# j-moralejo-pinas/dist_classicrl

Hardware: AMD Instinct MI355X
Metric: env-steps/sec at 128 agents, 1e6x16 Q-table; 1/2/4/8 GPU + HBM GB/s %peak (higher is better)
Workload: dtype f32

## Files before the change

dist_classicrl_amd/csrc/qe_rollout_df.h:

```cpp
#pragma once
#include "qe_rollout_lane.h"

namespace qe {

constexpr int DF_CAP = 128;
constexpr int DF_WT = 4096;
constexpr uint32_t DF_EMPTY = 0xFFFFFFFFu;
constexpr int64_t DF_MAX_STATES = 1ll << 25;
constexpr int DF_SPIN_LIMIT = 1 << 18;
constexpr unsigned ERR_DF_TIMEOUT = 5u;

struct M128 {
    unsigned long long lo, hi;
};
__device__ __forceinline__ M128 m128_zero() { return M128{0ull, 0ull}; }
__device__ __forceinline__ bool m128_any(const M128& a) { return (a.lo | a.hi) != 0ull; }
__device__ __forceinline__ M128 m128_and(const M128& a, const M128& b) { return M128{a.lo & b.lo, a.hi & b.hi}; }
__device__ __forceinline__ M128 m128_andnot(const M128& a, const M128& b) { return M128{a.lo & ~b.lo, a.hi & ~b.hi}; }
__device__ __forceinline__ M128 m128_or(const M128& a, const M128& b) { return M128{a.lo | b.lo, a.hi | b.hi}; }
__device__ __forceinline__ M128 m128_bit(int i) {
    return M128{i < 64 ? 1ull << i : 0ull, i >= 64 ? 1ull << (i - 64) : 0ull};
}
__device__ __forceinline__ M128 m128_below(int i) {
    return M128{i < 64 ? (1ull << i) - 1ull : ~0ull, i > 64 ? (1ull << (i - 64)) - 1ull : 0ull};
// ... 152 lines not shown
    const int tid = threadIdx.x;
    const int n_main = (int)((c.N + 63) & ~63ll);
    const int wave_tid = __builtin_amdgcn_readfirstlane(tid);
    const bool helper = wave_tid >= n_main;
    const int n_waves = n_main >> 6;
    const int i = helper ? tid - n_main : (tid & 63) * n_waves + (tid >> 6);
    const bool active = FULL ? !helper : (!helper && i < c.N);
    const int ii = i < c.N ? i : 0;
    Pending<T> p;
    p.n = helper ? 0 : c.n[ii];
    p.aux = c.aux[ii];
    p.s = 0; p.a = 0; p.pred = 0; p.r = 0.0f; p.term = false;
    float acc = c.acc[ii];
    unsigned long long dep_total = 0, ep_base = 0;
    unsigned extra_rounds = 0;
    int w_next = WT, w_cur = WT, w_prev = WT;
    int own_next = DF_CAP, own_cur = DF_CAP, own_prev = DF_CAP;
    const int flush_every = 32;
    int flush_in = flush_every;
    for (int k = tid; k < 4 * (WT + 1); k += (int)blockDim.x) (&lds.key[0][0])[k] = DF_EMPTY;
    for (int k = tid; k < 4 * (DF_CAP + 1) * 4; k += (int)blockDim.x) (&lds.wmask[0][0][0])[k] = 0u;
    for (int k = tid; k < 2 * DF_CAP; k += (int)blockDim.x) df_pub_write(&lds.pub[0][0] + k, 0u, (T)0, 0);
    static_assert(sizeof(Ctx<T>) <= sizeof(lds.cold), "context stash too small");
    if (tid == 0) {
        *reinterpret_cast<Ctx<T>*>(lds.cold) = c;
        lds.ep_n = 0u; lds.abort_ = 0u; lds.stat_dep = 0u; lds.stat_rounds = 0u;
        c.ctrl->error = 0u;
        c.ctrl->inv_count = 0u;
    }
    __syncthreads();
    const M128 my_bit = m128_bit(ii), below = m128_below(ii);
    const bool nan_sel = c.nan_select != 0;

    auto advance = [&](const RowV<T, NV>& row, M valid, long long t1, const U4& x, unsigned long long thr_t1, bool row_nan) {
        const bool explore = (unsigned long long)x.x < thr_t1;
        T picked;
        int act = select_lane<T, NV, M>(masked_row<MASKED>(row, valid), valid, explore, x.y, x.z, &picked, nan_sel && row_nan);
        if (act < 0) {
            c.ctrl->error = ERR_EMPTY_CHOICE;
            act = 0;
        }
        const int32_t n = p.n;
        const Transition tr = Env::step(ev, i, n, p.aux, act, c.step0 + (unsigned long long)t1);
        p.s = n; p.a = act; p.pred = picked; p.r = tr.reward; p.term = tr.terminated; p.n = tr.next_obs;
        lds.pub_a[t1 & 3][ii] = (unsigned char)act;
    };
    auto philox_of = [&](long long t1) {
        const unsigned long long step1 = c.step0 + (unsigned long long)t1;
        return philox4x32_10(c.agent_offset + (uint32_t)ii, (uint32_t)step1, (uint32_t)(step1 >> 32), STREAM_POLICY,
                             c.seed_lo, c.seed_hi);
    };
    auto draws = [&](long long t1) {
        const int slot = (int)(t1 & 1);
        return U4{lds.draws[slot][0][ii], lds.draws[slot][1][ii], lds.draws[slot][2][ii], 0u};
    };
    auto produce = [&](long long t1) {
        const U4 x = philox_of(t1);
        const int slot = (int)(t1 & 1);
        lds.draws[slot][0][ii] = x.x; lds.draws[slot][1][ii] = x.y; lds.draws[slot][2][ii] = x.z;
    };

    M128 Ws = my_bit;
    M128 Wn = m128_zero();
    M128 Wst = m128_zero();
    auto bookkeeping = [&](long long k, bool first) {
        uint32_t* const key_w = lds.key[(k + 1) & 3];
        const uint32_t* const key_r = lds.key[k & 3];
        const uint32_t* const key_st = lds.key[(k + 3) & 3];
        const uint32_t rowid = (uint32_t)p.n;
        const uint32_t mine = (rowid << 7) | (uint32_t)ii;
// ... 8 lines not shown
             odd_st = k_st != DF_EMPTY && (k_st >> 7) != rowid;
        while (__any(odd_w || odd_r || odd_st)) {
            h_w = odd_w ? (h_w + 1) & (WT - 1) : h_w;
            h_r = (h_r + 1) & (WT - 1);
            h_st = (h_st + 1) & (WT - 1);
            const uint32_t o2 = atomicCAS(&key_w[odd_w ? h_w : WT], odd_w ? DF_EMPTY : DF_EMPTY - 1u, mine);
            const uint32_t r2 = key_r[odd_r ? h_r : WT];
            const uint32_t s2 = key_st[odd_st ? h_st : WT];
            o_w = odd_w ? o2 : o_w; k_r = odd_r ? r2 : k_r; k_st = odd_st ? s2 : k_st;
            odd_w = o_w != DF_EMPTY && (o_w >> 7) != rowid; odd_r = k_r != DF_EMPTY && (k_r >> 7) != rowid;
            odd_st = k_st != DF_EMPTY && (k_st >> 7) != rowid;
        }
        const int own_w = o_w == DF_EMPTY ? ii : (int)(o_w & 127u);
        atomicOr(&lds.wmask[(k + 1) & 3][own_w][ii >> 5], 1u << (ii & 31));
        const bool found_r = k_r != DF_EMPTY, found_st = k_st != DF_EMPTY;
        Wn = m128_zero();
        Wst = m128_zero();
        if (__any(found_r || found_st)) {
            const M128 mr = lds_mask_load(lds.wmask[k & 3][found_r ? (int)(k_r & 127u) : DF_CAP]);
            const M128 ms = lds_mask_load(lds.wmask[(k + 3) & 3][found_st ? (int)(k_st & 127u) : DF_CAP]);
            if (found_r) Wn = mr;
            if (found_st) Wst = ms;
        }
        w_prev = w_cur; w_cur = w_next; w_next = h_w;
        own_prev = own_cur; own_cur = own_next; own_next = own_w;
    };

    RowV<T, NV> row;
    RowV<T, NV> row_next;
    {
        load_row_lane<NV>(row, c.q, p.n);
        if (active) {
            const M valid0 = valid_mask_lane<Env, NV, MASKED>(ev, i, p.n);
            advance(row, valid0, 0, philox_of(0), c.thr[0], row_nan_lane<NV>(masked_row<MASKED>(row, valid0)));
            const uint32_t rowid = (uint32_t)p.s, mine = (rowid << 7) | (uint32_t)ii;
            int h = (int)(mix32(rowid) & (WT - 1));
            uint32_t old = atomicCAS(&lds.key[0][h], DF_EMPTY, mine);
            while (old != DF_EMPTY && (old >> 7) != rowid) {
                h = (h + 1) & (WT - 1);
                old = atomicCAS(&lds.key[0][h], DF_EMPTY, mine);
            }
            own_next = old == DF_EMPTY ? ii : (int)(old & 127u);
            atomicOr(&lds.wmask[0][own_next][ii >> 5], 1u << (ii & 31));
            w_next = h;
        }
        if (helper) produce(1);
        __syncthreads();
        if (active) bookkeeping(0, true);
        load_row_lane<NV>(row_next, c.q, p.n);
        asm volatile("" ::: "memory");
        c.pred[ii] = (T)0;
        if constexpr (LEAN == 2) reinterpret_cast<DeltaEntry*>(c.pred)[ii] = DeltaEntry{0u, 0.0f};
    }
    __syncthreads();
    DeltaEntry* dl = c.dlog ? c.dlog + c.dlog_base + ii : nullptr;
    const long long dl_steps = c.dlog ? (c.dlog_cap - c.dlog_base) / c.N : 0;
    double lr_t = c.lr[0];
    unsigned long long thr_t1 = c.thr[steps > 1 ? 1 : 0];
    int vzero;
    asm volatile("v_mov_b32 %0, 0" : "=v"(vzero));
    bool timed_out = false;
    for (long long t = 0; t < steps; ++t) {
        const bool last = t + 1 == steps;
        const bool dl_ok = t < dl_steps;
        QL_STAMP(7);
        const U4 x = draws(t + 1);
        if (helper && !last) produce(t + 2);
        const uint32_t stamp = ((uint32_t)t + 1u) & 0xFFFFFFu, stamp_prev = (uint32_t)t & 0xFFFFFFu;
        const int par = (int)(t & 1);
        const M valid = valid_mask_lane<Env, NV, MASKED>(ev, ii, p.n);
        if constexpr (LEAN == 2) asm volatile("s_waitcnt vmcnt(2)" ::: "memory");
        else asm volatile("s_waitcnt vmcnt(1)" ::: "memory");
        df_take_row<T, NV>(row, row_next);
        const double lr_next = ((const double*)(uintptr_t)c.lr)[(last ? t : t + 1) + vzero];
        const unsigned long long thr_next = ((const unsigned long long*)(uintptr_t)c.thr)[(t + 2 < steps ? t + 2 : steps - 1) + vzero];
        const bool company = active && (m128_any(m128_andnot(Ws, my_bit)) || m128_any(Wn) || m128_any(Wst));
        const bool any_company = __any(company);
        const bool self_loop = p.n == p.s;
        const float r_t = p.r;
        const bool term_t = p.term;
        const int64_t cell = (int64_t)p.s * (4 * NV) + p.a;
        T q1 = 0, u = 0;
        bool row_nan = false;
        bool dep_u = false;
        bool is_last = active;
        QL_STAMP(0);
        float u_t = 0.0f;
        unsigned ep_raw = 0;
        unsigned long long enders = 0;
        float ep_value = 0.0f;
        auto body = [&](auto company_tag) {
            constexpr bool COMPANY = decltype(company_tag)::value;
            if constexpr (!COMPANY) {
                row_nan = row_nan_lane<NV>(masked_row<MASKED>(row, valid));
                if (active) {
                    T m = row_max_lane(masked_row<MASKED>(row, valid));
                    if (row_nan) m = quiet_nan<T>();
                    q1 = Td<T>::apply(p.pred, p.r, m, p.term, make_hyper(c, lr_t), 0, &u);
                    df_pub_write(&lds.pub[par][ii], stamp, q1, p.a);
                }
            } else {
                DfPub<T>* const pub_now = lds.pub[par];
                DfPub<T>* const pub_prev = lds.pub[par ^ 1];
                const unsigned char* const cols_now = lds.pub_a[t & 3];
                const unsigned char* const cols_prev = lds.pub_a[(t + 3) & 3];
                const M128 S_low = m128_and(Ws, below);
                const M128 N_low = p.term ? m128_zero() : (self_loop ? S_low : m128_and(Wn, below));
                dep_u = active && (m128_any(S_low) || m128_any(N_low));
                M128 hi = active ? m128_andnot(m128_andnot(Ws, below), my_bit) : m128_zero();
                const bool any_st = __any(active && m128_any(Wst)), any_dep = __any(dep_u), any_hi = __any(m128_any(hi));
                int j0 = -1, j1 = -1, cnt_st = 0;
                if (any_st) cnt_st = m128_two_lowest(active ? Wst : m128_zero(), &j0, &j1);
                int s0 = -1, s1 = -1, ns = 0, n0 = -1, n1 = -1, nn = 0;
                if (any_dep && dep_u) {
                    ns = m128_two_lowest(S_low, &s0, &s1);
                    nn = m128_two_lowest(N_low, &n0, &n1);
                }
                int h0 = -1, h1 = -1, nh = 0;
                if (any_hi) nh = m128_two_lowest(hi, &h0, &h1);
                T v0 = 0, v1 = 0;
                int c0 = 0, c1 = 0;
                unsigned long long raw_st0 = 0ull, raw_st1 = 0ull;
                if (any_st) {
                    if constexpr (sizeof(T) == 4) {
                        raw_st0 = df_pub_raw(pub_prev, j0 >= 0 ? j0 : ii);
                        raw_st1 = df_pub_raw(pub_prev, j1 >= 0 ? j1 : ii);
                    } else {
                        (void)df_pub_read(pub_prev, cols_prev, j0 >= 0 ? j0 : ii, stamp_prev, &v0, &c0);
                        (void)df_pub_read(pub_prev, cols_prev, j1 >= 0 ? j1 : ii, stamp_prev, &v1, &c1);
// ... 109 lines not shown
                }
                dep_total += dep_u ? 1ull : 0ull;
                if (any_hi) {
                    if (nh >= 1) is_last &= a_h0 != p.a;
                    if (nh >= 2) is_last &= a_h1 != p.a;
                    if (__any(nh > 2)) {
                        if (nh <= 2) hi = m128_zero();
                        while (m128_any(hi)) {
                            const int j = m128_pop_lowest(hi);
                            is_last &= (int)cols_now[j] != p.a;
                        }
                    }
                }
            }
            u_t = (float)u;
            QL_STAMP(2);
            if (active) {
                acc += r_t;
                enders = __ballot(term_t && (flags & FLAG_ACCOUNT));
                const unsigned rank = __builtin_amdgcn_mbcnt_hi((unsigned)(enders >> 32), __builtin_amdgcn_mbcnt_lo((unsigned)enders, 0u));
                if (term_t) {
                    if (rank == 0) ep_raw = atomicAdd(&lds.ep_n, (unsigned)__popcll(enders));
                    ep_value = acc;
                    acc = 0.0f;
                }
            }
            QL_STAMP(4);
            if (!last) {
                if constexpr (!COMPANY) {
                    if (__any(self_loop)) {
                        if (self_loop) {
                            row_set_lane<T, NV>(row, p.a, q1);
                            row_nan |= q1 != q1;
                        }
                    }
                } else {
                    DfPub<T>* const pub_now = lds.pub[par];
                    const unsigned char* const cols_now = lds.pub_a[t & 3];
                    const M128 others = m128_andnot(self_loop ? Ws : Wn, my_bit);
                    const bool dep_s = active && m128_any(others);
                    T v0 = 0, v1 = 0;
                    int c0 = 0, c1 = 0, j0 = -1, j1 = -1;
                    const int cnt = m128_two_lowest(others, &j0, &j1);
                    if (__any(dep_s)) {
                        for (int spin = 0; !timed_out; ++spin) {
                            bool ready = true;
                            if (dep_s) {
                                bool ok_0, ok_1;
                                df_pub_read2(pub_now, cols_now, j0 >= 0 ? j0 : ii, j1 >= 0 ? j1 : ii, stamp, &v0, &c0, &ok_0, &v1, &c1, &ok_1);
                                ready = (j0 < 0 || ok_0) && (j1 < 0 || ok_1);
                                if (cnt > 2) {
                                    M128 w = others;
                                    while (m128_any(w)) {
                                        const int j = m128_pop_lowest(w);
                                        T v;
                                        int col;
                                        ready &= df_pub_read(pub_now, cols_now, j, stamp, &v, &col);
                                    }
                                }
                            }
                            if (!__any(!ready)) break;
                            if (spin > DF_SPIN_LIMIT) { timed_out = true; lds.abort_ = 1u; }
                            __builtin_amdgcn_s_sleep(1);
                        }
                    }
                    if (dep_s && cnt <= 2) {
                        if (cnt >= 1) row_set_lane<T, NV>(row, c0, v0);
                        if (cnt >= 2) row_set_lane<T, NV>(row, c1, v1);
                        const bool mine_wins = self_loop && !((cnt >= 1 && j0 > ii && c0 == p.a) || (cnt >= 2 && j1 > ii && c1 == p.a));
                        if (__any(mine_wins)) {
                            if (mine_wins) row_set_lane<T, NV>(row, p.a, q1);
                        }
                    } else if (dep_s) {
                        M128 w = self_loop ? Ws : Wn;
                        while (m128_any(w)) {
                            const int j = m128_pop_lowest(w);
                            T v;
                            int col;
                            (void)df_pub_read(pub_now, cols_now, j, stamp, &v, &col);
                            row_set_lane<T, NV>(row, col, v);
                        }
                    } else if (active && self_loop) {
                        row_set_lane<T, NV>(row, p.a, q1);
                    }
                    row_nan = row_nan_lane<NV>(masked_row<MASKED>(row, valid));
                }
                if (active) advance(row, valid, t + 1, x, thr_t1, row_nan);
            }
        };
        if (any_company) body(std::true_type{});
        else body(std::false_type{});
        QL_STAMP(5);
        if (enders) {
            const unsigned base = __builtin_amdgcn_readlane(ep_raw, __ffsll((long long)enders) - 1);
            if ((enders >> (threadIdx.x & 63)) & 1) {
                const unsigned ep_slot = base + __builtin_amdgcn_mbcnt_hi((unsigned)(enders >> 32),
                                                                          __builtin_amdgcn_mbcnt_lo((unsigned)enders, 0u));
                const unsigned long long key = ((unsigned long long)t << 32) | (unsigned long long)i;
                if (ep_slot < (unsigned)EP_STAGE) {
                    lds.ep_key[ep_slot] = key;
                    lds.ep_ret[ep_slot] = ep_value;
                } else {
                    asm volatile("" ::: "memory");
                    const Ctx<T>& cc = *reinterpret_cast<const Ctx<T>*>(lds.cold);
                    if ((long long)(ep_base + ep_slot) < cc.ep_cap) {
                        cc.ep_key[ep_base + ep_slot] = key;
                        cc.ep_ret[ep_base + ep_slot] = ep_value;
                    }
                }
            }
        }
        bool leave = false;
        if (--flush_in == 0 || last) {
            flush_in = flush_every;
            __syncthreads();
            const unsigned staged = lds.ep_n;
            leave = lds.abort_ != 0u;
            const Ctx<T>& cc = *reinterpret_cast<const Ctx<T>*>(lds.cold);
            unsigned long long* const out_key = cc.ep_key;
            float* const out_ret = cc.ep_ret;
// ... 72 lines not shown
```

dist_classicrl_amd/csrc/qe_rollout_lane.h:

```cpp
#pragma once
#include "qe_kernels.h"

namespace qe {

constexpr int LANE_MAX_AGENTS = 512;

template <typename T, int NV>
struct RowV {
    T v[4 * NV];
};

template <int NV>
struct LaneMask {
    using type = uint32_t;
};
template <>
struct LaneMask<16> {
    using type = uint64_t;
};

__device__ __forceinline__ int popc_mask(uint32_t x) { return __popc(x); }
__device__ __forceinline__ int popc_mask(uint64_t x) { return __popcll(x); }

template <int NV>
__device__ __forceinline__ void load_row_lane(RowV<float, NV>& r, const float* q, int64_t row) {
    const float4* p = reinterpret_cast<const float4*>(q + row * (4 * NV));
#pragma unroll
    for (int k = 0; k < NV; ++k) {
        const float4 f = p[k];
        r.v[4 * k] = f.x; r.v[4 * k + 1] = f.y; r.v[4 * k + 2] = f.z; r.v[4 * k + 3] = f.w;
    }
}
template <int NV>
__device__ __forceinline__ void load_row_lane(RowV<double, NV>& r, const double* q, int64_t row) {
    const double2* p = reinterpret_cast<const double2*>(q + row * (4 * NV));
#pragma unroll
    for (int k = 0; k < NV; ++k) {
        const double2 a = p[2 * k], b = p[2 * k + 1];
        r.v[4 * k] = a.x; r.v[4 * k + 1] = a.y; r.v[4 * k + 2] = b.x; r.v[4 * k + 3] = b.y;
    }
}

__device__ __forceinline__ float lane_fmax(float a, float b) { return __builtin_fmaxf(a, b); }
__device__ __forceinline__ double lane_fmax(double a, double b) { return __builtin_fmax(a, b); }

template <bool MASKED, typename T, int NV, typename M>
__device__ __forceinline__ RowV<T, NV> masked_row(const RowV<T, NV>& row, M valid) {
    if constexpr (!MASKED) {
        return row;
    } else {
        RowV<T, NV> r;
#pragma unroll
// ... 28 lines not shown
__device__ __forceinline__ bool row_nan_lane(const RowV<double, NV>& rowm) {
    double acc = 0.0;
#pragma unroll
    for (int j = 0; j < 4 * NV; ++j) acc += rowm.v[j] * rowm.v[j];
    return acc != acc;
}
template <typename T, int NV>
__device__ __forceinline__ T row_max_np_lane(const RowV<T, NV>& rowm) {
    const T m = row_max_lane(rowm);
    return row_nan_lane<NV>(rowm) ? quiet_nan<T>() : m;
}

template <typename T, int NV, int LO, int CNT>
__device__ __forceinline__ T row_pick_tree(const RowV<T, NV>& row, int idx) {
    constexpr int W = 4 * NV;
    if constexpr (CNT == 1) {
        T x = row.v[LO < W ? LO : W - 1];
        asm volatile("" : "+v"(x));
        return x;
    } else {
        const T lo = row_pick_tree<T, NV, LO, CNT / 2>(row, idx);
        const T hi = row_pick_tree<T, NV, LO + CNT / 2, CNT / 2>(row, idx);
        T r = (idx & (CNT / 2)) ? hi : lo;
        asm volatile("" : "+v"(r));
        return r;
    }
}
template <typename T, int NV>
__device__ __forceinline__ T row_pick_lane(const RowV<T, NV>& row, int idx) {
    constexpr int W = 4 * NV;
    constexpr int P = W <= 4 ? 4 : (W <= 8 ? 8 : (W <= 16 ? 16 : (W <= 32 ? 32 : 64)));
    return row_pick_tree<T, NV, 0, P>(row, idx);
}

template <int NV, typename M>
__device__ __forceinline__ int kth_set_bit(M f, int k) {
    constexpr int W = 4 * NV;
    constexpr int P = W <= 4 ? 4 : (W <= 8 ? 8 : (W <= 16 ? 16 : (W <= 32 ? 32 : 64)));
    constexpr int LOG = P == 4 ? 2 : (P == 8 ? 3 : (P == 16 ? 4 : (P == 32 ? 5 : 6)));
    int pos = 0;
#pragma unroll
    for (int lv = 0; lv < LOG; ++lv) {
        const int width = P >> (lv + 1);
        const M low = f & (((M)1 << width) - 1);
        const int c = popc_mask(low);
        const bool hi = k >= c;
        k -= hi ? c : 0;
        f = hi ? (f >> width) : low;
        pos += hi ? width : 0;
    }
    return pos;
}

template <typename T, int NV, typename M>
__device__ __forceinline__ int select_lane(const RowV<T, NV>& rowm, M valid, bool explore, uint32_t x1,
                                           uint32_t x2, T* picked, bool nan_max) {
    T m = row_max_lane(rowm);
    if (nan_max) m = quiet_nan<T>();
    M ties = 0;
#pragma unroll
    for (int j = 0; j < 4 * NV; ++j) ties |= (M)(rowm.v[j] == m ? 1u : 0u) << j;
    const M f = explore ? valid : (ties & valid);
    const int total = popc_mask(f);
    int act = -1;
    if (total > 0) act = kth_set_bit<NV>(f, (int)mulhi32(explore ? x1 : x2, (uint32_t)total));
    *picked = row_pick_lane(rowm, act < 0 ? 0 : act);
    return act;
}

template <class Env, int NV, bool MASKED>
__device__ __forceinline__ typename LaneMask<NV>::type valid_mask_lane(const EnvCtx& ev, int64_t i, int32_t obs) {
    using M = typename LaneMask<NV>::type;
    if constexpr (!MASKED) {
        return ev.A >= 8 * (int)sizeof(M) ? ~(M)0 : (((M)1 << ev.A) - 1);
    } else {
        M m = 0;
#pragma unroll
        for (int sub = 0; sub < NV; ++sub) m |= (M)Env::valid4(ev, i, obs, sub) << (4 * sub);
        return m;
    }
}

template <int CAP>
struct LaneCfg {
    static constexpr int WT = CAP <= 128 ? 4096 : 2048;
    static constexpr int BT = 2048;
};

template <int CAP, bool HELP>
struct LaneLds {
    SlowLdsT<CAP, PERSIST_CACHE_BYTES> slow;
    int wt[4][LaneCfg<CAP>::WT + 1];
    int bt_key[LaneCfg<CAP>::BT];
    unsigned bt_cnt[LaneCfg<CAP>::BT];
    int bt_min[LaneCfg<CAP>::BT];
    uint32_t draws[2][3][HELP ? CAP : 1];
    unsigned long long ep_key[EP_STAGE];
    float ep_ret[EP_STAGE];
    unsigned char pending[CAP];
    alignas(16) unsigned char cold[448];
    unsigned def_bits[CAP / 32];
    unsigned busy[5];
    unsigned ep_n;
    unsigned n_def;
    unsigned complex_;
    int seq_min[2];
};

#ifdef QE_EXPERIMENT
#define QX(bit) ((flags >> (20 + (bit))) & 1)
#else
#define QX(bit) 0
#endif
#ifdef QE_STAMPS
#define QL_STAMP(k) do { const long long _n = wall_clock64(); stamp_sum[k] += _n - stamp_last; stamp_last = _n; } while (0)
#else
#define QL_STAMP(k) do { } while (0)
#endif

template <int PENDING_LOADS>
__device__ __forceinline__ void step_barrier() {
    if constexpr (PENDING_LOADS == 0) asm volatile("s_waitcnt vmcnt(0) lgkmcnt(0)\n\ts_barrier" ::: "memory");
    else asm volatile("s_waitcnt vmcnt(%0) lgkmcnt(0)\n\ts_barrier" ::"n"(PENDING_LOADS) : "memory");
}

template <typename T, class Env, int NV, int CAP, bool MASKED, int LEAN = 0, bool HELP = false, bool FULL = false,
          bool SEQ = false>
__global__ __launch_bounds__(HELP ? 4 * CAP : CAP) void k_rollout_lane(InlineSched ,
                                                                       Ctx<T> c, EnvCtx ev, long long steps, int flags) {
    using M = typename LaneMask<NV>::type;
    constexpr int NLOAD = NV * (int)(sizeof(T) / 4);
    constexpr int WT = LaneCfg<CAP>::WT, BT = LaneCfg<CAP>::BT;
    __shared__ LaneLds<CAP, HELP> lds;
    const unsigned long long clk0 = wall_clock64();
    const unsigned long long cyc0 = __builtin_amdgcn_s_memtime();
    if (c.thr == nullptr) {
        const QE_AS4 unsigned char* ka = (const QE_AS4 unsigned char*)__builtin_amdgcn_kernarg_segment_ptr();
        c.thr = (const QE_AS4 unsigned long long*)ka;
        c.lr = (const QE_AS4 double*)(ka + sizeof(unsigned long long) * INLINE_SCHED_STEPS);
    }
    if constexpr (LEAN != 0) { c.mode = 0; c.trace = nullptr; c.rp.s = nullptr; }
    if constexpr (LEAN == 1) c.dlog = nullptr;
#ifdef QE_STAMPS
    long long stamp_sum[8] = {0, 0, 0, 0, 0, 0, 0, 0};
    long long stamp_last = wall_clock64();
    if (threadIdx.x == 0) for (int k = 8; k < 24; ++k) c.vinc[k] = 0.0;
#endif
    const int tid = threadIdx.x;
    const int n_main = HELP ? (int)((c.N + 63) & ~63ll) : (int)blockDim.x;
    const int wave_tid = __builtin_amdgcn_readfirstlane(tid);
    const bool helper = HELP && wave_tid >= n_main && wave_tid < 2 * n_main;
    const bool worker = HELP && wave_tid >= 2 * n_main;
    const int i = helper ? tid - n_main : (worker ? 0 : tid);
    const bool active = FULL ? !(helper || worker) : (!(helper || worker) && i < c.N);
    const int ii = i < c.N ? i : 0;
    Pending<T> p;
    p.n = c.n[ii];
    p.aux = c.aux[ii];
    p.s = 0; p.a = 0; p.pred = 0; p.r = 0.0f; p.term = false;
    float acc = c.acc[ii];
    unsigned long long deferred_total = 0, ep_base = 0;
    unsigned complex_steps = 0;
    int w_next = WT, w_cur = WT, w_prev = WT;
    const int flush_every = 32;
    int flush_in = flush_every;
    for (int k = tid; k < 4 * (WT + 1); k += (int)blockDim.x) (&lds.wt[0][0])[k] = -1;
    for (int k = tid; k < BT; k += (int)blockDim.x) { lds.bt_key[k] = -1; lds.bt_cnt[k] = 0u; lds.bt_min[k] = 0x7FFFFFFF; }
    for (int k = tid; k < CAP; k += (int)blockDim.x) lds.pending[k] = 0;
    if (tid < CAP / 32) lds.def_bits[tid] = 0u;
    static_assert(sizeof(Ctx<T>) <= sizeof(lds.cold), "context stash too small");
    if (tid == 0) {
        *reinterpret_cast<Ctx<T>*>(lds.cold) = c;
        lds.ep_n = 0u; lds.n_def = 0u; lds.complex_ = 0u;
        lds.seq_min[0] = 0x7FFFFFFF; lds.seq_min[1] = 0x7FFFFFFF;
        for (int k = 0; k < 5; ++k) lds.busy[k] = 0u;
        c.ctrl->error = 0u;
        c.ctrl->inv_count = 0u;
    }
    __syncthreads();
    if ((QX(6) && worker) || (QX(7) && helper)) return;

    const bool nan_sel = c.nan_select != 0;
    auto advance = [&](const RowV<T, NV>& row, M valid, long long t1, const U4& x, unsigned long long thr_t1, bool row_nan) {
        const bool explore = (unsigned long long)x.x < thr_t1;
        T picked;
        int act = select_lane<T, NV, M>(masked_row<MASKED>(row, valid), valid, explore, x.y, x.z, &picked, nan_sel && row_nan);
        if (act < 0) {
            c.ctrl->error = ERR_EMPTY_CHOICE;
            act = 0;
        }
        const int32_t n = p.n;
        const Transition tr = Env::step(ev, i, n, p.aux, act, c.step0 + (unsigned long long)t1);
        if (c.trace) c.trace[t1 * c.N + i] = act;
        replay_put(c, t1, i, n, act, tr.reward, tr.next_obs, tr.terminated);
        p.s = n; p.a = act; p.pred = picked; p.r = tr.reward; p.term = tr.terminated; p.n = tr.next_obs;
    };
    auto philox_of = [&](long long t1) {
        const unsigned long long step1 = c.step0 + (unsigned long long)t1;
        return philox4x32_10(c.agent_offset + (uint32_t)ii, (uint32_t)step1, (uint32_t)(step1 >> 32), STREAM_POLICY,
                             c.seed_lo, c.seed_hi);
    };
    auto draws = [&](long long t1) {
        if constexpr (HELP) {
            const int slot = (int)(t1 & 1);
            return U4{lds.draws[slot][0][ii], lds.draws[slot][1][ii], lds.draws[slot][2][ii], 0u};
        } else {
            return philox_of(t1);
        }
    };
    auto produce = [&](long long t1) {
        const U4 x = philox_of(t1);
        const int slot = (int)(t1 & 1);
        lds.draws[slot][0][ii] = x.x; lds.draws[slot][1][ii] = x.y; lds.draws[slot][2][ii] = x.z;
    };
    auto bookkeeping = [&](long long k, bool check_stale) {
        int* const tab_w = lds.wt[(k + 1) & 3];
        const int* const tab_r = lds.wt[k & 3];
        const int* const tab_st = lds.wt[(k + 3) & 3];
        const int32_t rowid = p.n;
        const int h = (int)(mix32((uint32_t)rowid) & (WT - 1));
        const bool need_r = rowid != p.s;
        int o_w = atomicCAS(&tab_w[h], -1, rowid);
        int k_r = need_r ? tab_r[h] : -1;
        int k_st = check_stale ? tab_st[h] : -1;
        int h_w = h, h_r = h, h_st = h;
        bool odd_w = o_w != -1 && o_w != rowid, odd_r = k_r != -1 && k_r != rowid, odd_st = k_st != -1 && k_st != rowid;
        while (__any(odd_w || odd_r || odd_st)) {
            h_w = odd_w ? (h_w + 1) & (WT - 1) : h_w;
            h_r = (h_r + 1) & (WT - 1);
            h_st = (h_st + 1) & (WT - 1);
            const int o2 = atomicCAS(&tab_w[odd_w ? h_w : WT], odd_w ? -1 : -2, rowid);
            const int r2 = tab_r[odd_r ? h_r : WT];
            const int s2 = tab_st[odd_st ? h_st : WT];
            o_w = odd_w ? o2 : o_w; k_r = odd_r ? r2 : k_r; k_st = odd_st ? s2 : k_st;
            odd_w = o_w != -1 && o_w != rowid; odd_r = k_r != -1 && k_r != rowid; odd_st = k_st != -1 && k_st != rowid;
        }
        lds.busy[o_w == rowid ? (int)((k + 1) & 3) : 4] = 1u;
        lds.busy[k_r == rowid ? (int)(k & 3) : 4] = 1u;
        w_prev = w_cur; w_cur = w_next; w_next = h_w;
        return k_st == rowid;
    };

    RowV<T, NV> row;
    bool stale = false;
    {
        load_row_lane<NV>(row, c.q, p.n);
        if (active) {
            const M valid0 = valid_mask_lane<Env, NV, MASKED>(ev, i, p.n);
            advance(row, valid0, 0, philox_of(0), c.thr[0], row_nan_lane<NV>(masked_row<MASKED>(row, valid0)));
            int h = (int)(mix32((uint32_t)p.s) & (WT - 1));
            int old = atomicCAS(&lds.wt[0][h], -1, p.s);
            while (old != -1 && old != p.s) {
                h = (h + 1) & (WT - 1);
                old = atomicCAS(&lds.wt[0][h], -1, p.s);
            }
            if (old == p.s) lds.busy[0] = 1u;
            w_next = h;
        }
        if (helper) produce(1);
        __syncthreads();
        if (active) (void)bookkeeping(0, false);
        load_row_lane<NV>(row, c.q, p.n);
    }
    __syncthreads();
    DeltaEntry* dl = c.dlog ? c.dlog + c.dlog_base + ii : nullptr;
    const long long dl_steps = c.dlog ? (c.dlog_cap - c.dlog_base) / c.N : 0;
    int vzero;
    asm volatile("v_mov_b32 %0, 0" : "=v"(vzero));
    double lr_pend = ((const double*)(uintptr_t)c.lr)[vzero];
    unsigned long long thr_pend = ((const unsigned long long*)(uintptr_t)c.thr)[(steps > 1 ? 1 : 0) + vzero];
    for (long long t = 0; t < steps; ++t) {
        const bool last = t + 1 == steps;
        const bool dl_ok = t < dl_steps;
        QL_STAMP(7);
        const bool busy = lds.busy[t & 3] != 0u;
        const U4 x = draws(t + 1);
        if (helper && !last && !QX(5)) produce(t + 2);
        if (stale && !QX(8)) load_row_lane<NV>(row, c.q, p.n);
        const M valid = valid_mask_lane<Env, NV, MASKED>(ev, ii, p.n);
        QL_STAMP(0);
        int cls = 3;
        int pred_s = -1, pred_n = -1;
        int b_s = -1, b_n = -1;
        if (busy) {
            if (active) {
                auto bt_insert = [&](int32_t rowid) {
                    int h = (int)(mix32((uint32_t)rowid) & (BT - 1));
                    for (;;) {
                        const int old = atomicCAS(&lds.bt_key[h], -1, rowid);
                        if (old == -1 || old == rowid) return h;
                        h = (h + 1) & (BT - 1);
                    }
                };
                b_s = bt_insert(p.s);
                atomicAdd(&lds.bt_cnt[b_s], 1u << 16);
                atomicMin(&lds.bt_min[b_s], i);
                if (p.n != p.s) {
                    b_n = bt_insert(p.n);
                    atomicAdd(&lds.bt_cnt[b_n], 1u);
                    atomicMin(&lds.bt_min[b_n], i);
                }
            }
            barrier_lds();
            if (active) {
                const unsigned cs = lds.bt_cnt[b_s];
                const int ms = lds.bt_min[b_s];
                unsigned cn = 0u;
                int mn = 0x7FFFFFFF;
                const bool has_n = b_n >= 0;
                if (has_n) { cn = lds.bt_cnt[b_n]; mn = lds.bt_min[b_n]; }
                const unsigned w_s = cs >> 16, tot_s = w_s + (cs & 0xFFFFu);
                const unsigned w_n = cn >> 16, tot_n = w_n + (cn & 0xFFFFu);
                bool now = true, sel = true, cx = false;
                if (c.mode == 1) {
                    const bool shared = w_s >= 2u || (w_s == 1u && tot_s >= 2u) || (has_n && w_n >= 1u && tot_n >= 2u);
                    if (shared) { now = false; cx = true; }
                    sel = !(has_n ? w_n > 0u : w_s > 1u);
                } else {
                    if (tot_s > 1u && ms < i) { now = false; pred_s = ms; cx |= tot_s > 2u; }
                    if (has_n) {
                        if (w_n > 0u) {
                            sel = false;
                            if (!p.term && mn < i) { now = false; pred_n = mn; cx |= tot_n > 2u; }
                        }
                    } else if (w_s > 1u) {
                        sel = false;
                    }
                }
                cls = (now ? 1 : 0) | (sel ? 2 : 0);
                if (!now) {
                    lds.pending[i] = 1;
                    atomicAdd(&lds.n_def, 1u);
                    if (cx) lds.complex_ = 1u;
                }
            }
        }
        QL_STAMP(2);
        __builtin_amdgcn_s_waitcnt(0x0F70);
        double lr_t;
        unsigned long long thr_t1;
        asm volatile("v_mov_b64 %0, %1" : "=v"(lr_t) : "v"(lr_pend));
        asm volatile("v_mov_b64 %0, %1" : "=v"(thr_t1) : "v"(thr_pend));
        lr_pend = ((const double*)(uintptr_t)c.lr)[(last ? t : t + 1) + vzero];
        thr_pend = ((const unsigned long long*)(uintptr_t)c.thr)[(t + 2 < steps ? t + 2 : steps - 1) + vzero];
        const float r_t = p.r;
        const bool term_t = p.term;
        bool row_nan = row_nan_lane<NV>(masked_row<MASKED>(row, valid));
        if (active && (cls & 1)) {
            T m = row_max_lane(masked_row<MASKED>(row, valid));
            if (row_nan) m = quiet_nan<T>();
            const int64_t cell = (int64_t)p.s * (4 * NV) + p.a;
            T u;
            const T q1 = Td<T>::apply(p.pred, p.r, m, p.term, make_hyper(c, lr_t), c.mode, &u);
            if (p.n == p.s) row_nan |= q1 != q1;
            if (!QX(1)) c.q[cell] = q1;
            if (dl_ok) *dl = DeltaEntry{(uint32_t)cell, (float)u};
            if (p.n == p.s) {
#pragma unroll
                for (int j = 0; j < 4 * NV; ++j) row.v[j] = j == p.a ? q1 : row.v[j];
            }
        }
        unsigned ep_raw = 0;
        unsigned long long enders = 0;
        float ep_value = 0.0f;
        if (active) {
            acc += r_t;
            enders = __ballot(term_t && (flags & FLAG_ACCOUNT));
            const unsigned rank = __builtin_amdgcn_mbcnt_hi((unsigned)(enders >> 32), __builtin_amdgcn_mbcnt_lo((unsigned)enders, 0u));
            if (term_t) {
                if (rank == 0) ep_raw = atomicAdd(&lds.ep_n, (unsigned)__popcll(enders));
                ep_value = acc;
                acc = 0.0f;
            }
        }
        QL_STAMP(4);
        if (active && !busy && !last) advance(row, valid, t + 1, x, thr_t1, row_nan);
        QL_STAMP(5);

        if (busy) {
#ifdef QE_STAMPS
            const long long ext_t0 = wall_clock64();
#endif
            __syncthreads();
            const int n_def = (int)lds.n_def;
            if (active) {
                lds.bt_key[b_s] = -1; lds.bt_cnt[b_s] = 0u; lds.bt_min[b_s] = 0x7FFFFFFF;
                if (b_n >= 0) { lds.bt_key[b_n] = -1; lds.bt_cnt[b_n] = 0u; lds.bt_min[b_n] = 0x7FFFFFFF; }
            }
#ifdef QE_STAMPS
            if (tid == 0) { c.vinc[16] += 1.0; if (n_def > 0) c.vinc[17] += 1.0; }
#endif
            if (n_def > 0) {
                deferred_total += (unsigned long long)n_def;
                if (lds.complex_) ++complex_steps;
                if constexpr (SEQ) if (lds.complex_) {
                    bool mine = active && !(cls & 1);
                    for (int round = 0; round <= n_def; ++round) {
                        if (mine) atomicMin(&lds.seq_min[round & 1], i);
                        barrier_lds();
                        const int turn = lds.seq_min[round & 1];
                        if (tid == 0) lds.seq_min[(round + 1) & 1] = 0x7FFFFFFF;
                        if (turn == 0x7FFFFFFF) break;
                        if (mine && i == turn) {
                            T m = 0;
                            if (!p.term) {
                                RowV<T, NV> fresh;
                                load_row_lane<NV>(fresh, c.q, p.n);
                                m = row_max_np_lane<T, NV>(masked_row<MASKED>(fresh, valid));
                            }
// ... 47 lines not shown
                } else if (!lds.complex_) {
                    bool mine = active && !(cls & 1);
                    int rounds = 0;
                    while (lds.n_def > 0u && rounds++ <= n_def) {
#ifdef QE_STAMPS
                        if (tid == 0) c.vinc[18] += 1.0;
#endif
                        const bool go = mine && (pred_s < 0 || lds.pending[pred_s] == 0) &&
                                        (pred_n < 0 || lds.pending[pred_n] == 0);
                        barrier_lds();
                        if (go) {
                            T m = 0;
                            if (!p.term) {
                                RowV<T, NV> fresh;
                                load_row_lane<NV>(fresh, c.q, p.n);
                                m = row_max_np_lane<T, NV>(masked_row<MASKED>(fresh, valid));
                            }
                            const int64_t cell = (int64_t)p.s * (4 * NV) + p.a;
                            const T q0 = c.q[cell];
                            T u;
                            c.q[cell] = Td<T>::apply(q0, p.r, m, p.term, make_hyper(c, lr_t), 0, &u);
                            log_delta(c, t, i, cell, u);
                            lds.pending[i] = 0;
                            atomicSub(&lds.n_def, 1u);
                            mine = false;
                        }
                        __syncthreads();
                    }
                    if (tid == 0 && lds.n_def > 0u) reinterpret_cast<const Ctx<T>*>(lds.cold)->ctrl->error = 2u;
                }
            }
            if (active && !last) {
                if (cls != 3 && !((cls & 2) && p.n != p.s)) load_row_lane<NV>(row, c.q, p.n);
                advance(row, valid, t + 1, x, thr_t1, row_nan_lane<NV>(masked_row<MASKED>(row, valid)));
            }
            if (tid == 0) { lds.n_def = 0u; lds.complex_ = 0u; }
            __builtin_amdgcn_s_waitcnt(0x0F70);
#ifdef QE_STAMPS
            if (tid == 0) c.vinc[19] += (double)(wall_clock64() - ext_t0);
#endif
        }
        if (enders) {
            const unsigned base = __builtin_amdgcn_readlane(ep_raw, __ffsll((long long)enders) - 1);
            if ((enders >> (threadIdx.x & 63)) & 1) {
                const unsigned ep_slot = base + __builtin_amdgcn_mbcnt_hi((unsigned)(enders >> 32),
                                                                          __builtin_amdgcn_mbcnt_lo((unsigned)enders, 0u));
                const unsigned long long key = ((unsigned long long)t << 32) | (unsigned long long)i;
                if (ep_slot < (unsigned)EP_STAGE) {
                    lds.ep_key[ep_slot] = key;
                    lds.ep_ret[ep_slot] = ep_value;
                } else {
                    asm volatile("" ::: "memory");
                    const Ctx<T>& cc = *reinterpret_cast<const Ctx<T>*>(lds.cold);
                    if ((long long)(ep_base + ep_slot) < cc.ep_cap) {
                        cc.ep_key[ep_base + ep_slot] = key;
                        cc.ep_ret[ep_base + ep_slot] = ep_value;
                    }
                }
            }
        }
        if (--flush_in == 0 || last) {
            flush_in = flush_every;
            __syncthreads();
            const unsigned staged = lds.ep_n;
            const Ctx<T>& cc = *reinterpret_cast<const Ctx<T>*>(lds.cold);
            unsigned long long* const out_key = cc.ep_key;
            float* const out_ret = cc.ep_ret;
            const long long out_cap = cc.ep_cap;
            for (unsigned k = tid; k < min(staged, (unsigned)EP_STAGE); k += blockDim.x) {
                const unsigned long long pos = ep_base + k;
                if ((long long)pos < out_cap) { out_key[pos] = lds.ep_key[k]; out_ret[pos] = lds.ep_ret[k]; }
            }
            ep_base += staged;
            __syncthreads();
            if (tid == 0) lds.ep_n = 0u;
// ... 49 lines not shown
```

Baseline: 29.16 million.

## Micro-optimize lane rollout step with inline-asm picks, tie masks, reused row max

Adds several independently toggleable micro-optimizations to the per-lane rollout loop. Row pick and tie-mask construction are replaced with hand-written cndmask/addc inline assembly. The row max already computed for the TD target is passed into action selection instead of being recomputed, and the episode counter increment uses a raw ds_add_rtn with a deferred waitcnt. Accounting and the row-landed wait are moved ahead of the busy-flag read so the LDS read latency can overlap with other work. Hand-written assembly adds register pressure and correctness risk, and the NaN and tie semantics must still match the generic path.

```diff
diff --git a/dist_classicrl_amd/csrc/qe_rollout_df.h b/dist_classicrl_amd/csrc/qe_rollout_df.h
--- a/dist_classicrl_amd/csrc/qe_rollout_df.h
+++ b/dist_classicrl_amd/csrc/qe_rollout_df.h
@@ -208,10 +208,12 @@
     const M128 my_bit = m128_bit(ii), below = m128_below(ii);
     const bool nan_sel = c.nan_select != 0;
 
-    auto advance = [&](const RowV<T, NV>& row, M valid, long long t1, const U4& x, unsigned long long thr_t1, bool row_nan) {
+    auto advance = [&](const RowV<T, NV>& row, M valid, long long t1, const U4& x, unsigned long long thr_t1, bool row_nan,
+                       const T* row_max) {
         const bool explore = (unsigned long long)x.x < thr_t1;
         T picked;
-        int act = select_lane<T, NV, M>(masked_row<MASKED>(row, valid), valid, explore, x.y, x.z, &picked, nan_sel && row_nan);
+        int act = select_lane<T, NV, M>(masked_row<MASKED>(row, valid), valid, explore, x.y, x.z, &picked, nan_sel && row_nan,
+                                        row_max);
         if (act < 0) {
             c.ctrl->error = ERR_EMPTY_CHOICE;
             act = 0;
@@ -286,7 +288,7 @@
         load_row_lane<NV>(row, c.q, p.n);
         if (active) {
             const M valid0 = valid_mask_lane<Env, NV, MASKED>(ev, i, p.n);
-            advance(row, valid0, 0, philox_of(0), c.thr[0], row_nan_lane<NV>(masked_row<MASKED>(row, valid0)));
+            advance(row, valid0, 0, philox_of(0), c.thr[0], row_nan_lane<NV>(masked_row<MASKED>(row, valid0)), nullptr);
             const uint32_t rowid = (uint32_t)p.s, mine = (rowid << 7) | (uint32_t)ii;
             int h = (int)(mix32(rowid) & (WT - 1));
             uint32_t old = atomicCAS(&lds.key[0][h], DF_EMPTY, mine);
@@ -345,10 +347,12 @@
         float ep_value = 0.0f;
         auto body = [&](auto company_tag) {
             constexpr bool COMPANY = decltype(company_tag)::value;
+            T m_sel = neg_inf<T>();
             if constexpr (!COMPANY) {
                 row_nan = row_nan_lane<NV>(masked_row<MASKED>(row, valid));
                 if (active) {
                     T m = row_max_lane(masked_row<MASKED>(row, valid));
+                    m_sel = m;
                     if (row_nan) m = quiet_nan<T>();
                     q1 = Td<T>::apply(p.pred, p.r, m, p.term, make_hyper(c, lr_t), 0, &u);
                     df_pub_write(&lds.pub[par][ii], stamp, q1, p.a);
@@ -524,6 +528,9 @@
                         if (self_loop) {
                             row_set_lane<T, NV>(row, p.a, q1);
                             row_nan |= q1 != q1;
+#if QE_LANE_ONE_ROW_MAX
+                            m_sel = row_max_lane(masked_row<MASKED>(row, valid));
+#endif
                         }
                     }
                 } else {
@@ -577,7 +584,7 @@
                     }
                     row_nan = row_nan_lane<NV>(masked_row<MASKED>(row, valid));
                 }
-                if (active) advance(row, valid, t + 1, x, thr_t1, row_nan);
+                if (active) advance(row, valid, t + 1, x, thr_t1, row_nan, (QE_LANE_ONE_ROW_MAX && !COMPANY) ? &m_sel : nullptr);
             }
         };
         if (any_company) body(std::true_type{});
diff --git a/dist_classicrl_amd/csrc/qe_rollout_lane.h b/dist_classicrl_amd/csrc/qe_rollout_lane.h
--- a/dist_classicrl_amd/csrc/qe_rollout_lane.h
+++ b/dist_classicrl_amd/csrc/qe_rollout_lane.h
@@ -18,6 +18,22 @@
 struct LaneMask<16> {
     using type = uint64_t;
 };
+
+#ifndef QE_LANE_TIE_CARRY
+#define QE_LANE_TIE_CARRY 1
+#endif
+#ifndef QE_LANE_PICK_BLOCK
+#define QE_LANE_PICK_BLOCK 1
+#endif
+#ifndef QE_LANE_ONE_ROW_MAX
+#define QE_LANE_ONE_ROW_MAX 1
+#endif
+#ifndef QE_LANE_EP_PLAIN_ATOMIC
+#define QE_LANE_EP_PLAIN_ATOMIC 1
+#endif
+#ifndef QE_LANE_BUSY_LATE
+#define QE_LANE_BUSY_LATE 1
+#endif
 
 __device__ __forceinline__ int popc_mask(uint32_t x) { return __popc(x); }
 __device__ __forceinline__ int popc_mask(uint64_t x) { return __popcll(x); }
@@ -112,6 +128,126 @@
     constexpr int P = W <= 4 ? 4 : (W <= 8 ? 8 : (W <= 16 ? 16 : (W <= 32 ? 32 : 64)));
     return row_pick_tree<T, NV, 0, P>(row, idx);
 }
+#if QE_LANE_PICK_BLOCK
+#define QE_PICK_SEL(d, a, b, s) "v_cndmask_b32_e64 %[" #d "], %[" #a "], %[" #b "], %[" #s "]\n\t"
+#define QE_PICK_SEL0(d, a, b) "v_cndmask_b32_e32 %[" #d "], %[" #a "], %[" #b "], vcc\n\t"
+template <>
+__device__ __forceinline__ float row_pick_lane<float, 4>(const RowV<float, 4>& row, int idx) {
+    float r, t1, t2, t3;
+    unsigned long long s1, s2, s3;
+    asm volatile(
+        "v_lshlrev_b32_e32 %[t1], 31, %[idx]\n\t"
+        "v_lshlrev_b32_e32 %[t2], 30, %[idx]\n\t"
+        "v_lshlrev_b32_e32 %[t3], 29, %[idx]\n\t"
+        "v_cmp_gt_i32_e32 vcc, 0, %[t1]\n\t"
+        "v_cmp_gt_i32_e64 %[s1], 0, %[t2]\n\t"
+        "v_cmp_gt_i32_e64 %[s2], 0, %[t3]\n\t"
+        "v_cmp_lt_u32_e64 %[s3], 7, %[idx]\n\t"
+        QE_PICK_SEL0(r, c0, c1) QE_PICK_SEL0(t1, c2, c3) QE_PICK_SEL(r, r, t1, s1)
+        QE_PICK_SEL0(t1, c4, c5) QE_PICK_SEL0(t2, c6, c7) QE_PICK_SEL(t1, t1, t2, s1)
+        QE_PICK_SEL(r, r, t1, s2)
+        QE_PICK_SEL0(t1, c8, c9) QE_PICK_SEL0(t2, c10, c11) QE_PICK_SEL(t1, t1, t2, s1)
+        QE_PICK_SEL0(t2, c12, c13) QE_PICK_SEL0(t3, c14, c15) QE_PICK_SEL(t2, t2, t3, s1)
+        QE_PICK_SEL(t1, t1, t2, s2)
+        "v_cndmask_b32_e64 %[r], %[r], %[t1], %[s3]"
+        : [r] "=&v"(r), [t1] "=&v"(t1), [t2] "=&v"(t2), [t3] "=&v"(t3), [s1] "=&s"(s1), [s2] "=&s"(s2), [s3] "=&s"(s3)
+        : [idx] "v"(idx), [c0] "v"(row.v[0]), [c1] "v"(row.v[1]), [c2] "v"(row.v[2]), [c3] "v"(row.v[3]),
+          [c4] "v"(row.v[4]), [c5] "v"(row.v[5]), [c6] "v"(row.v[6]), [c7] "v"(row.v[7]), [c8] "v"(row.v[8]),
+          [c9] "v"(row.v[9]), [c10] "v"(row.v[10]), [c11] "v"(row.v[11]), [c12] "v"(row.v[12]), [c13] "v"(row.v[13]),
+          [c14] "v"(row.v[14]), [c15] "v"(row.v[15])
+        : "vcc");
+    return r;
+}
+template <>
+__device__ __forceinline__ float row_pick_lane<float, 2>(const RowV<float, 2>& row, int idx) {
+    float r, t1, t2;
+    unsigned long long s1, s2;
+    asm volatile(
+        "v_lshlrev_b32_e32 %[t1], 31, %[idx]\n\t"
+        "v_lshlrev_b32_e32 %[t2], 30, %[idx]\n\t"
+        "v_cmp_gt_i32_e32 vcc, 0, %[t1]\n\t"
+        "v_cmp_gt_i32_e64 %[s1], 0, %[t2]\n\t"
+        "v_cmp_lt_u32_e64 %[s2], 3, %[idx]\n\t"
+        QE_PICK_SEL0(r, c0, c1) QE_PICK_SEL0(t1, c2, c3) QE_PICK_SEL(r, r, t1, s1)
+        QE_PICK_SEL0(t1, c4, c5) QE_PICK_SEL0(t2, c6, c7) QE_PICK_SEL(t1, t1, t2, s1)
+        "v_cndmask_b32_e64 %[r], %[r], %[t1], %[s2]"
+        : [r] "=&v"(r), [t1] "=&v"(t1), [t2] "=&v"(t2), [s1] "=&s"(s1), [s2] "=&s"(s2)
+        : [idx] "v"(idx), [c0] "v"(row.v[0]), [c1] "v"(row.v[1]), [c2] "v"(row.v[2]), [c3] "v"(row.v[3]),
+          [c4] "v"(row.v[4]), [c5] "v"(row.v[5]), [c6] "v"(row.v[6]), [c7] "v"(row.v[7])
+        : "vcc");
+    return r;
+}
+#undef QE_PICK_SEL
+#undef QE_PICK_SEL0
+#endif
+
+template <typename T, int NV, typename M>
+__device__ __forceinline__ M tie_mask_lane(const RowV<T, NV>& rowm, T m) {
+    M ties = 0;
+#pragma unroll
+    for (int j = 0; j < 4 * NV; ++j) ties |= (M)(rowm.v[j] == m ? 1u : 0u) << j;
+    return ties;
+}
+#if QE_LANE_TIE_CARRY
+#define QE_TIE_CMP(p, c) "v_cmp_eq_f32_e64 %[" #p "], %[" #c "], %[m]\n\t"
+#define QE_TIE_ADD(p) "v_addc_co_u32_e64 %[acc], %[" #p "], %[acc], %[acc], %[" #p "]\n\t"
+#define QE_TIE_CMP0(c) "v_cmp_eq_f32_e32 vcc, %[" #c "], %[m]\n\t"
+#define QE_TIE_ADD0 "v_addc_co_u32_e32 %[acc], vcc, %[acc], %[acc], vcc\n\t"
+template <>
+__device__ __forceinline__ uint32_t tie_mask_lane<float, 4, uint32_t>(const RowV<float, 4>& rowm, float m) {
+    uint32_t acc;
+    unsigned long long p1, p2;
+    asm volatile(
+        QE_TIE_CMP0(c15) QE_TIE_CMP(p1, c14) QE_TIE_CMP(p2, c13)
+        "v_cndmask_b32_e64 %[acc], 0, 1, vcc\n\t"
+        QE_TIE_CMP0(c12) QE_TIE_ADD(p1)
+        QE_TIE_CMP(p1, c11) QE_TIE_ADD(p2)
+        QE_TIE_CMP(p2, c10) QE_TIE_ADD0
+        QE_TIE_CMP0(c9) QE_TIE_ADD(p1)
+        QE_TIE_CMP(p1, c8) QE_TIE_ADD(p2)
+        QE_TIE_CMP(p2, c7) QE_TIE_ADD0
+        QE_TIE_CMP0(c6) QE_TIE_ADD(p1)
+        QE_TIE_CMP(p1, c5) QE_TIE_ADD(p2)
+        QE_TIE_CMP(p2, c4) QE_TIE_ADD0
+        QE_TIE_CMP0(c3) QE_TIE_ADD(p1)
+        QE_TIE_CMP(p1, c2) QE_TIE_ADD(p2)
+        QE_TIE_CMP(p2, c1) QE_TIE_ADD0
+        QE_TIE_CMP0(c0) QE_TIE_ADD(p1)
+        QE_TIE_ADD(p2)
+        "v_addc_co_u32_e32 %[acc], vcc, %[acc], %[acc], vcc"
+        : [acc] "=&v"(acc), [p1] "=&s"(p1), [p2] "=&s"(p2)
+        : [m] "v"(m), [c0] "v"(rowm.v[0]), [c1] "v"(rowm.v[1]), [c2] "v"(rowm.v[2]), [c3] "v"(rowm.v[3]),
+          [c4] "v"(rowm.v[4]), [c5] "v"(rowm.v[5]), [c6] "v"(rowm.v[6]), [c7] "v"(rowm.v[7]), [c8] "v"(rowm.v[8]),
+          [c9] "v"(rowm.v[9]), [c10] "v"(rowm.v[10]), [c11] "v"(rowm.v[11]), [c12] "v"(rowm.v[12]),
+          [c13] "v"(rowm.v[13]), [c14] "v"(rowm.v[14]), [c15] "v"(rowm.v[15])
+        : "vcc");
+    return acc;
+}
+template <>
+__device__ __forceinline__ uint32_t tie_mask_lane<float, 2, uint32_t>(const RowV<float, 2>& rowm, float m) {
+    uint32_t acc;
+    unsigned long long p1, p2;
+    asm volatile(
+        QE_TIE_CMP0(c7) QE_TIE_CMP(p1, c6) QE_TIE_CMP(p2, c5)
+        "v_cndmask_b32_e64 %[acc], 0, 1, vcc\n\t"
+        QE_TIE_CMP0(c4) QE_TIE_ADD(p1)
+        QE_TIE_CMP(p1, c3) QE_TIE_ADD(p2)
+        QE_TIE_CMP(p2, c2) QE_TIE_ADD0
+        QE_TIE_CMP0(c1) QE_TIE_ADD(p1)
+        QE_TIE_CMP(p1, c0) QE_TIE_ADD(p2)
+        QE_TIE_ADD0
+        "v_addc_co_u32_e64 %[acc], %[p1], %[acc], %[acc], %[p1]"
+        : [acc] "=&v"(acc), [p1] "=&s"(p1), [p2] "=&s"(p2)
+        : [m] "v"(m), [c0] "v"(rowm.v[0]), [c1] "v"(rowm.v[1]), [c2] "v"(rowm.v[2]), [c3] "v"(rowm.v[3]),
+          [c4] "v"(rowm.v[4]), [c5] "v"(rowm.v[5]), [c6] "v"(rowm.v[6]), [c7] "v"(rowm.v[7])
+        : "vcc");
+    return acc;
+}
+#undef QE_TIE_CMP
+#undef QE_TIE_ADD
+#undef QE_TIE_CMP0
+#undef QE_TIE_ADD0
+#endif
 
 template <int NV, typename M>
 __device__ __forceinline__ int kth_set_bit(M f, int k) {
@@ -134,12 +270,10 @@
 
 template <typename T, int NV, typename M>
 __device__ __forceinline__ int select_lane(const RowV<T, NV>& rowm, M valid, bool explore, uint32_t x1,
-                                           uint32_t x2, T* picked, bool nan_max) {
-    T m = row_max_lane(rowm);
+                                           uint32_t x2, T* picked, bool nan_max, const T* row_max = nullptr) {
+    T m = row_max ? *row_max : row_max_lane(rowm);
     if (nan_max) m = quiet_nan<T>();
-    M ties = 0;
-#pragma unroll
-    for (int j = 0; j < 4 * NV; ++j) ties |= (M)(rowm.v[j] == m ? 1u : 0u) << j;
+    const M ties = tie_mask_lane<T, NV, M>(rowm, m);
     const M f = explore ? valid : (ties & valid);
     const int total = popc_mask(f);
     int act = -1;
@@ -198,6 +332,11 @@
 #define QL_STAMP(k) do { } while (0)
 #endif
 
+template <typename P>
+__device__ __forceinline__ uint32_t lds_offset(P* p) {
+    return (uint32_t)(uintptr_t)(__attribute__((address_space(3))) void*)p;
+}
+
 template <int PENDING_LOADS>
 __device__ __forceinline__ void step_barrier() {
     if constexpr (PENDING_LOADS == 0) asm volatile("s_waitcnt vmcnt(0) lgkmcnt(0)\n\ts_barrier" ::: "memory");
@@ -211,6 +350,7 @@
     using M = typename LaneMask<NV>::type;
     constexpr int NLOAD = NV * (int)(sizeof(T) / 4);
     constexpr int WT = LaneCfg<CAP>::WT, BT = LaneCfg<CAP>::BT;
+    constexpr bool EP_ASM = QE_LANE_EP_PLAIN_ATOMIC && LEAN != 0 && SEQ;
     __shared__ LaneLds<CAP, HELP> lds;
     const unsigned long long clk0 = wall_clock64();
     const unsigned long long cyc0 = __builtin_amdgcn_s_memtime();
@@ -261,10 +401,12 @@
     if ((QX(6) && worker) || (QX(7) && helper)) return;
 
     const bool nan_sel = c.nan_select != 0;
-    auto advance = [&](const RowV<T, NV>& row, M valid, long long t1, const U4& x, unsigned long long thr_t1, bool row_nan) {
+    auto advance = [&](const RowV<T, NV>& row, M valid, long long t1, const U4& x, unsigned long long thr_t1, bool row_nan,
+                       const T* row_max) {
         const bool explore = (unsigned long long)x.x < thr_t1;
         T picked;
-        int act = select_lane<T, NV, M>(masked_row<MASKED>(row, valid), valid, explore, x.y, x.z, &picked, nan_sel && row_nan);
+        int act = select_lane<T, NV, M>(masked_row<MASKED>(row, valid), valid, explore, x.y, x.z, &picked, nan_sel && row_nan,
+                                        row_max);
         if (act < 0) {
             c.ctrl->error = ERR_EMPTY_CHOICE;
             act = 0;
@@ -327,7 +469,7 @@
         load_row_lane<NV>(row, c.q, p.n);
         if (active) {
             const M valid0 = valid_mask_lane<Env, NV, MASKED>(ev, i, p.n);
-            advance(row, valid0, 0, philox_of(0), c.thr[0], row_nan_lane<NV>(masked_row<MASKED>(row, valid0)));
+            advance(row, valid0, 0, philox_of(0), c.thr[0], row_nan_lane<NV>(masked_row<MASKED>(row, valid0)), nullptr);
             int h = (int)(mix32((uint32_t)p.s) & (WT - 1));
             int old = atomicCAS(&lds.wt[0][h], -1, p.s);
             while (old != -1 && old != p.s) {
@@ -349,15 +491,65 @@
     asm volatile("v_mov_b32 %0, 0" : "=v"(vzero));
     double lr_pend = ((const double*)(uintptr_t)c.lr)[vzero];
     unsigned long long thr_pend = ((const unsigned long long*)(uintptr_t)c.thr)[(steps > 1 ? 1 : 0) + vzero];
+#if QE_LANE_BUSY_LATE
+    asm volatile("" : "+v"(acc));
+#endif
     for (long long t = 0; t < steps; ++t) {
         const bool last = t + 1 == steps;
         const bool dl_ok = t < dl_steps;
         QL_STAMP(7);
-        const bool busy = lds.busy[t & 3] != 0u;
+        const unsigned busy_raw = lds.busy[t & 3];
         const U4 x = draws(t + 1);
         if (helper && !last && !QX(5)) produce(t + 2);
         if (stale && !QX(8)) load_row_lane<NV>(row, c.q, p.n);
         const M valid = valid_mask_lane<Env, NV, MASKED>(ev, ii, p.n);
+        double lr_t;
+        unsigned long long thr_t1;
+        bool row_nan = false;
+        T m_row = neg_inf<T>();
+        auto row_landed = [&]() {
+            __builtin_amdgcn_s_waitcnt(0x0F70);
+            asm volatile("v_mov_b64 %0, %1" : "=v"(lr_t) : "v"(lr_pend));
+            asm volatile("v_mov_b64 %0, %1" : "=v"(thr_t1) : "v"(thr_pend));
+            lr_pend = ((const double*)(uintptr_t)c.lr)[(last ? t : t + 1) + vzero];
+            thr_pend = ((const unsigned long long*)(uintptr_t)c.thr)[(t + 2 < steps ? t + 2 : steps - 1) + vzero];
+            row_nan = row_nan_lane<NV>(masked_row<MASKED>(row, valid));
+#if QE_LANE_BUSY_LATE
+            m_row = row_max_lane(masked_row<MASKED>(row, valid));
+#endif
+        };
+        unsigned ep_raw = 0;
+        unsigned long long enders = 0;
+        float ep_value = 0.0f;
+        const float r_t = p.r;
+        const bool term_t = p.term;
+        auto account = [&]() {
+            if (active) {
+                acc += r_t;
+                enders = __ballot(term_t && (flags & FLAG_ACCOUNT));
+                const unsigned rank = __builtin_amdgcn_mbcnt_hi((unsigned)(enders >> 32), __builtin_amdgcn_mbcnt_lo((unsigned)enders, 0u));
+                if (term_t) {
+                    if constexpr (EP_ASM) {
+                        if (rank == 0) {
+                            asm volatile("ds_add_rtn_u32 %0, %1, %2" : "+v"(ep_raw) : "v"(lds_offset(&lds.ep_n)), "v"((unsigned)__popcll(enders)) : "memory");
+                        }
+                    } else {
+                        if (rank == 0) ep_raw = atomicAdd(&lds.ep_n, (unsigned)__popcll(enders));
+                    }
+                    ep_value = acc;
+                    acc = 0.0f;
+                }
+            }
+        };
+#if QE_LANE_BUSY_LATE
+        account();
+        row_landed();
+        unsigned busy_v = busy_raw;
+        asm volatile("" : "+v"(busy_v) : "v"(m_row), "v"(x.x), "v"(x.y), "v"(x.z));
+        const bool busy = __builtin_amdgcn_readfirstlane(busy_v) != 0u;
+#else
+        const bool busy = busy_raw != 0u;
+#endif
         QL_STAMP(0);
         int cls = 3;
         int pred_s = -1, pred_n = -1;
@@ -416,18 +608,16 @@
             }
         }
         QL_STAMP(2);
-        __builtin_amdgcn_s_waitcnt(0x0F70);
-        double lr_t;
-        unsigned long long thr_t1;
-        asm volatile("v_mov_b64 %0, %1" : "=v"(lr_t) : "v"(lr_pend));
-        asm volatile("v_mov_b64 %0, %1" : "=v"(thr_t1) : "v"(thr_pend));
-        lr_pend = ((const double*)(uintptr_t)c.lr)[(last ? t : t + 1) + vzero];
-        thr_pend = ((const unsigned long long*)(uintptr_t)c.thr)[(t + 2 < steps ? t + 2 : steps - 1) + vzero];
-        const float r_t = p.r;
-        const bool term_t = p.term;
-        bool row_nan = row_nan_lane<NV>(masked_row<MASKED>(row, valid));
+#if !QE_LANE_BUSY_LATE
+        row_landed();
+#endif
+        T m_sel = m_row;
         if (active && (cls & 1)) {
-            T m = row_max_lane(masked_row<MASKED>(row, valid));
+#if !QE_LANE_BUSY_LATE
+            m_row = row_max_lane(masked_row<MASKED>(row, valid));
+#endif
+            T m = m_row;
+            m_sel = m;
             if (row_nan) m = quiet_nan<T>();
             const int64_t cell = (int64_t)p.s * (4 * NV) + p.a;
             T u;
@@ -438,23 +628,16 @@
             if (p.n == p.s) {
 #pragma unroll
                 for (int j = 0; j < 4 * NV; ++j) row.v[j] = j == p.a ? q1 : row.v[j];
-            }
-        }
-        unsigned ep_raw = 0;
-        unsigned long long enders = 0;
-        float ep_value = 0.0f;
-        if (active) {
-            acc += r_t;
-            enders = __ballot(term_t && (flags & FLAG_ACCOUNT));
-            const unsigned rank = __builtin_amdgcn_mbcnt_hi((unsigned)(enders >> 32), __builtin_amdgcn_mbcnt_lo((unsigned)enders, 0u));
-            if (term_t) {
-                if (rank == 0) ep_raw = atomicAdd(&lds.ep_n, (unsigned)__popcll(enders));
-                ep_value = acc;
-                acc = 0.0f;
-            }
-        }
+#if QE_LANE_ONE_ROW_MAX
+                m_sel = row_max_lane(masked_row<MASKED>(row, valid));
+#endif
+            }
+        }
+#if !QE_LANE_BUSY_LATE
+        account();
+#endif
         QL_STAMP(4);
-        if (active && !busy && !last) advance(row, valid, t + 1, x, thr_t1, row_nan);
+        if (active && !busy && !last) advance(row, valid, t + 1, x, thr_t1, row_nan, QE_LANE_ONE_ROW_MAX ? &m_sel : nullptr);
         QL_STAMP(5);
 
         if (busy) {
@@ -568,7 +751,7 @@
             }
             if (active && !last) {
                 if (cls != 3 && !((cls & 2) && p.n != p.s)) load_row_lane<NV>(row, c.q, p.n);
-                advance(row, valid, t + 1, x, thr_t1, row_nan_lane<NV>(masked_row<MASKED>(row, valid)));
+                advance(row, valid, t + 1, x, thr_t1, row_nan_lane<NV>(masked_row<MASKED>(row, valid)), nullptr);
             }
             if (tid == 0) { lds.n_def = 0u; lds.complex_ = 0u; }
             __builtin_amdgcn_s_waitcnt(0x0F70);
@@ -577,6 +760,7 @@
 #endif
         }
         if (enders) {
+            if constexpr (EP_ASM) asm volatile("s_waitcnt lgkmcnt(0)" : "+v"(ep_raw) : : "memory");
             const unsigned base = __builtin_amdgcn_readlane(ep_raw, __ffsll((long long)enders) - 1);
             if ((enders >> (threadIdx.x & 63)) & 1) {
                 const unsigned ep_slot = base + __builtin_amdgcn_mbcnt_hi((unsigned)(enders >> 32),
```

New measurement: 30.51 million, median of 5. +4.6%, better.
